# Tarseus/eam-rl4co

Measured on AMD Instinct MI355X. Metric: env-steps/sec (batch x num_loc / s), AttentionModel construction rollout, higher is better.
Workload: dtype f32; 1 GPU; TSP num_loc=100 batch=1024/GPU AM greedy rollout (encoder + cache + decode loop + reward); global_batch=1024, launch=hipGraph replay

## Files before the change

eam_rl4co_amd/csrc/encoder_fused.hip:

```cpp
#include "encoder_fused.hpp"

namespace eamrl {

constexpr int SA = 140;
constexpr int GA = 34;
constexpr int SQ = 66;

struct ALayout {
    float* HB;
    static constexpr int S = SA;
    __device__ float* col(int c) const { return HB + (c & 3) * GA + (c >> 2); }
    __device__ void store4(int row, int q4, float4 v) const
    {
        float* p = HB + row * SA + q4;
        p[0] = v.x; p[GA] = v.y; p[2 * GA] = v.z; p[3 * GA] = v.w;
    }
    __device__ float4 load4(int row, int q4) const
    {
        const float* p = HB + row * SA + q4;
        return make_float4(p[0], p[GA], p[2 * GA], p[3 * GA]);
    }
    __device__ void mirror(int, int, float) const {}
};

#ifdef EAMRL_STAMPS
__device__ unsigned long long g_enc_stamps[24];
#define ESTAMP(i) do { const unsigned long long now_ = __builtin_readcyclecounter(); st_acc[i] += now_ - st_t; st_t = now_; } while (0)
#else
#define ESTAMP(i) do { } while (0)
#endif

__device__ __forceinline__ f32x4 mfma4(float a, float b, f32x4 c) { return __builtin_amdgcn_mfma_f32_16x16x4f32(a, b, c, 0, 0, 0); }

typedef float f32x2v __attribute__((ext_vector_type(2)));
__device__ __forceinline__ float2 lds_read_b64(const float* p)
{
    typedef const volatile __attribute__((address_space(3))) f32x2v* lds_ptr;
    const f32x2v v = *(lds_ptr)(p);
    return make_float2(v.x, v.y);
}

template <int CT>
__device__ __forceinline__ void load_b0(float4 (&b0)[CT], const float* const (&wp)[CT])
{
#pragma unroll
    for (int ct = 0; ct < CT; ++ct) b0[ct] = *reinterpret_cast<const float4*>(wp[ct]);
}

template <int RTW, int CT, int S, bool SWAP, int NRT>
__device__ __forceinline__ void gemm_pass_n(f32x4 (&acc)[RTW][CT], const float* arow, const float* const (&wp)[CT],
                                            int NU, const float4 (&b0)[CT])
{
    constexpr int nrt = NRT;
    float4 bn[CT];
    float2 an0[RTW], an1[RTW];
#pragma unroll
    for (int ct = 0; ct < CT; ++ct) bn[ct] = b0[ct];
#pragma unroll
    for (int rt = 0; rt < RTW; ++rt)
        if (rt < nrt) {
            an0[rt] = lds_read_b64(arow + rt * 16 * S);
            an1[rt] = lds_read_b64(arow + rt * 16 * S + 2);
        }
    for (int u = 0; u < NU; ++u) {
        float4 b[CT];
        float2 a0[RTW], a1[RTW];
#pragma unroll
        for (int ct = 0; ct < CT; ++ct) b[ct] = bn[ct];
#pragma unroll
        for (int rt = 0; rt < RTW; ++rt) { a0[rt] = an0[rt]; a1[rt] = an1[rt]; }
        if (u + 1 < NU) {
#pragma unroll
            for (int ct = 0; ct < CT; ++ct) bn[ct] = *reinterpret_cast<const float4*>(wp[ct] + (u + 1) * 256);
#pragma unroll
            for (int rt = 0; rt < RTW; ++rt)
                if (rt < nrt) {
                    an0[rt] = lds_read_b64(arow + rt * 16 * S + 4 * (u + 1));
                    an1[rt] = lds_read_b64(arow + rt * 16 * S + 4 * (u + 1) + 2);
                }
        }
#pragma unroll
        for (int rt = 0; rt < RTW; ++rt)
            if (rt < nrt) {
#pragma unroll
                for (int ct = 0; ct < CT; ++ct)
                    acc[rt][ct] = SWAP ? mfma4(b[ct].x, a0[rt].x, acc[rt][ct]) : mfma4(a0[rt].x, b[ct].x, acc[rt][ct]);
#pragma unroll
                for (int ct = 0; ct < CT; ++ct)
                    acc[rt][ct] = SWAP ? mfma4(b[ct].y, a0[rt].y, acc[rt][ct]) : mfma4(a0[rt].y, b[ct].y, acc[rt][ct]);
#pragma unroll
                for (int ct = 0; ct < CT; ++ct)
                    acc[rt][ct] = SWAP ? mfma4(b[ct].z, a1[rt].x, acc[rt][ct]) : mfma4(a1[rt].x, b[ct].z, acc[rt][ct]);
#pragma unroll
                for (int ct = 0; ct < CT; ++ct)
                    acc[rt][ct] = SWAP ? mfma4(b[ct].w, a1[rt].y, acc[rt][ct]) : mfma4(a1[rt].y, b[ct].w, acc[rt][ct]);
            }
    }
}

template <int RTW, int CT, int S, bool SWAP = false, int NLOW = RTW>
__device__ __forceinline__ void gemm_pass(f32x4 (&acc)[RTW][CT], const float* arow, int nrt, const float* const (&wp)[CT],
                                          int NU, const float4 (&b0)[CT])
{
    if (NLOW == RTW || nrt == RTW) gemm_pass_n<RTW, CT, S, SWAP, RTW>(acc, arow, wp, NU, b0);
    else gemm_pass_n<RTW, CT, S, SWAP, NLOW>(acc, arow, wp, NU, b0);
}

template <int RTW>
__device__ __forceinline__ void residual_norm_store(const f32x4 (&acc)[RTW][2], float* HB, int row0, int nrt, int cw, int j, int G,
                                                    int norm, const float* cst )
{
#pragma unroll
    for (int ct = 0; ct < 2; ++ct) {
        const int c = 32 * cw + 16 * ct + j;
        const float sc = cst[c], sh = cst[FE + c];
        float* col = HB + (c & 3) * GA + (c >> 2);
#pragma unroll
        for (int rt = 0; rt < RTW; ++rt)
            if (rt < nrt) {
#pragma unroll
                for (int r = 0; r < 4; ++r) {
                    float* p = col + (row0 + 16 * rt + 4 * G + r) * SA;
                    float v = *p + acc[rt][ct][r];
                    if (norm == EAMRL_NORM_BATCH_EVAL) v = fma_(v, sc, sh);
                    *p = v;
                }
            }
    }
}

template <int RTT>
__global__ __launch_bounds__(512, 2) void k_encoder_fused(FusedArgs a)
{
    constexpr int RTA = (RTT + 1) / 2;
    constexpr int RTW = RTA;
    constexpr int ROWS = 16 * RTT;
    constexpr int SV = ROWS + 4;
    extern __shared__ __attribute__((aligned(16))) float lds[];
    float* HB = lds;
    float* QA = HB + ROWS * SA;
    float* KB = QA + ROWS * SQ;
    float* VT = KB + ROWS * SQ;
    float* HID = QA;
    float* CST = VT + 64 * SV;
    static_assert(ROWS * SA <= 2 * ROWS * SQ + 64 * SV, "HID must fit QA | KB | VT");
    const ALayout L{HB};

    const int tid = threadIdx.x, lane = tid & 63;
    const int wv = __builtin_amdgcn_readfirstlane(tid >> 6);
    const int cw = wv & 3, rw = wv >> 2;
    const int j = lane & 15, G = lane >> 4;
    const int M = a.M;
    const int row0 = rw ? 16 * RTA : 0;
    const int nrt = rw ? RTT - RTA : RTA;
    const int64_t inst = blockIdx.x;
#ifdef EAMRL_STAMPS
    unsigned long long st_acc[20] = {0, 0, 0, 0, 0, 0, 0, 0, 0, 0, 0, 0, 0, 0, 0, 0, 0, 0, 0, 0}, st_t = __builtin_readcyclecounter();
#endif

    if (a.h_in) load_h<ROWS>(a.h_in, M, L);
    else init_embedding<ROWS>(a.init, M, L);
    __syncthreads();
    ESTAMP(0);

    for (int layer = 0; layer < a.nlayers; ++layer) {
        const eamrl_encoder_layer& Ly = a.L[layer];
        for (int i = tid; i < NCST; i += blockDim.x) {
            float v;
            if (i < C_BO) v = Ly.bqkv[i];
            else if (i < C_B1) v = Ly.bo[i - C_BO];
            else if (i < C_B2) v = Ly.b1[i - C_B1];
            else if (i < C_N1) v = Ly.b2[i - C_B2];
            else {
                const bool second = i >= C_N2;
                const int k = (i - (second ? C_N2 : C_N1));
                const int c = k & (FE - 1);
                const float* gam = second ? Ly.n2_gamma : Ly.n1_gamma;
                const float* bet = second ? Ly.n2_beta : Ly.n1_beta;
                if (a.norm == EAMRL_NORM_BATCH_EVAL) {
                    const float* mean = second ? Ly.n2_mean : Ly.n1_mean;
                    const float* var = second ? Ly.n2_var : Ly.n1_var;
                    const float sc = gam[c] / __builtin_sqrtf(var[c] + a.eps);
                    const float ms = mean[c] * sc;
                    v = k < FE ? sc : bet[c] - ms;
                } else {
                    v = k < FE ? gam[c] : bet[c];
                }
            }
            CST[i] = v;
        }
        __syncthreads();
        f32x4 acc_o[RTW][2];
#pragma unroll
        for (int ct = 0; ct < 2; ++ct) {
            const float b = CST[C_BO + 32 * cw + 16 * ct + j];
#pragma unroll
            for (int rt = 0; rt < RTW; ++rt) acc_o[rt][ct] = splat4(b);
        }
        for (int hg = 0; hg < 2; ++hg) {
            const float* wp3[2];
            float4 b3[2];
#pragma unroll
            for (int ct = 0; ct < 2; ++ct)
                wp3[ct] = Ly.Wo + ((int64_t)(2 * cw + ct) * (FE / 16) + 4 * hg) * 256 + lane * 4;
            {
                f32x4 acc[RTW][3];
                const int ctq = 4 * hg + cw;
                const float* wp[3];
                float4 b0[3];
#pragma unroll
                for (int x = 0; x < 3; ++x) wp[x] = Ly.Wqkv + ((int64_t)(8 * x + ctq) * (FE / 16)) * 256 + lane * 4;
                load_b0<3>(b0, wp);
#pragma unroll
                for (int x = 0; x < 3; ++x) {
                    const float b = CST[C_BQKV + 16 * (8 * x + ctq) + j];
#pragma unroll
                    for (int rt = 0; rt < RTW; ++rt) acc[rt][x] = splat4(b);
                }
                ESTAMP(16);
                gemm_pass<RTW, 3, SA, false, RTT - RTA>(acc, HB + (row0 + j) * SA + G * GA, nrt, wp, FE / 16, b0);
                ESTAMP(17);
                load_b0<2>(b3, wp3);
                float* qcol = QA + (j & 3) * 16 + 4 * cw + (j >> 2);
                float* kcol = KB + (j & 3) * 16 + 4 * cw + (j >> 2);
                float* vrow = VT + (16 * cw + j) * SV;
#pragma unroll
                for (int rt = 0; rt < RTW; ++rt)
                    if (rt < nrt) {
                        const int rbase = row0 + 16 * rt + 4 * G;
#pragma unroll
                        for (int r = 0; r < 4; ++r) {
                            qcol[(rbase + r) * SQ] = acc[rt][0][r] * 0.25f;
                            kcol[(rbase + r) * SQ] = acc[rt][1][r];
                        }
                        *reinterpret_cast<float4*>(vrow + rbase) =
                            make_float4(acc[rt][2][0], acc[rt][2][1], acc[rt][2][2], acc[rt][2][3]);
                    }
            }
            ESTAMP(1);
            __syncthreads();
            ESTAMP(2);
            {
                const int pi = 4 * (j & 3) + (j >> 2);
                float kf[RTT][4];
#pragma unroll
                for (int kt = 0; kt < RTT; ++kt) {
                    const float* p = KB + (16 * kt + pi) * SQ + G * 16 + 4 * cw;
                    const float2 lo = *reinterpret_cast<const float2*>(p), hi = *reinterpret_cast<const float2*>(p + 2);
                    kf[kt][0] = lo.x; kf[kt][1] = lo.y; kf[kt][2] = hi.x; kf[kt][3] = hi.y;
                }
                float vf[4 * RTT];
                const int NT = (M + 3) >> 2;
                constexpr int FULLT = RTT == 7 ? 4 : RTT == 4 ? 2 : 0;
#pragma unroll
                for (int t = 0; t < 4 * RTT; ++t) vf[t] = (t < NT) ? VT[(16 * cw + j) * SV + 4 * t + G] : 0.0f;
                for (int q = 0; q < nrt; ++q) {
                    const int qrow = row0 + 16 * q + j;
                    const float* qp = QA + qrow * SQ + G * 16 + 4 * cw;
                    const float2 qlo = *reinterpret_cast<const float2*>(qp), qhi = *reinterpret_cast<const float2*>(qp + 2);
                    f32x4 s[RTT];
                    float m = -INFINITY;
#pragma unroll
                    for (int kt = 0; kt < RTT; ++kt) s[kt] = mfma4(kf[kt][0], qlo.x, splat4(0.0f));
#pragma unroll
                    for (int kt = 0; kt < RTT; ++kt) s[kt] = mfma4(kf[kt][1], qlo.y, s[kt]);
#pragma unroll
                    for (int kt = 0; kt < RTT; ++kt) s[kt] = mfma4(kf[kt][2], qhi.x, s[kt]);
#pragma unroll
                    for (int kt = 0; kt < RTT; ++kt) s[kt] = mfma4(kf[kt][3], qhi.y, s[kt]);
#pragma unroll
                    for (int kt = 0; kt < RTT; ++kt) {
                        if (kt >= FULLT && 16 * kt + 16 > M) {
#pragma unroll
                            for (int r = 0; r < 4; ++r)
                                if (16 * kt + 4 * r + G >= M) s[kt][r] = -INFINITY;
                        }
                        m = vmax5_raw(m, s[kt][0], s[kt][1], s[kt][2], s[kt][3]);
                    }
                    {
                        auto r16 = __builtin_amdgcn_permlane16_swap(__float_as_uint(m), __float_as_uint(m), false, false);
                        m = vmax_raw(__uint_as_float(r16[0]), __uint_as_float(r16[1]));
                        auto r32 = __builtin_amdgcn_permlane32_swap(__float_as_uint(m), __float_as_uint(m), false, false);
                        m = vmax_raw(__uint_as_float(r32[0]), __uint_as_float(r32[1]));
                    }
#pragma unroll
                    for (int kt = 0; kt < RTT; ++kt) {
                        f32x2 e01 = (f32x2){s[kt][0], s[kt][1]} - splat2(m), e23 = (f32x2){s[kt][2], s[kt][3]} - splat2(m);
                        d_expf2_nonpos_x2(e01, e23);
                        s[kt] = (f32x4){e01.x, e01.y, e23.x, e23.y};
                    }
                    float zp = s[0][0];
#pragma unroll
                    for (int t = 1; t < 4 * RTT; ++t) zp = zp + s[t >> 2][t & 3];
                    {
                        auto r16 = __builtin_amdgcn_permlane16_swap(__float_as_uint(zp), __float_as_uint(zp), false, false);
                        zp = __uint_as_float(r16[0]) + __uint_as_float(r16[1]);
                        auto r32 = __builtin_amdgcn_permlane32_swap(__float_as_uint(zp), __float_as_uint(zp), false, false);
                        zp = __uint_as_float(r32[0]) + __uint_as_float(r32[1]);
                    }
                    f32x4 o = splat4(0.0f);
#pragma unroll
                    for (int kt = 0; kt < RTT; ++kt)
                        if (kt < FULLT || 16 * kt < M) {
#pragma unroll
                            for (int r = 0; r < 4; ++r) o = mfma4(vf[4 * kt + r], s[kt][r], o);
                        }
                    float* op = QA + qrow * SQ + 4 * cw + G;
#pragma unroll
                    for (int r = 0; r < 4; ++r) op[r * 16] = o[r] / zp;
                }
            }
            ESTAMP(3);
            __syncthreads();
            ESTAMP(4);
            gemm_pass<RTW, 2, SQ, false, RTT - RTA>(acc_o, QA + (row0 + j) * SQ + G * 16, nrt, wp3, 4, b3);
            ESTAMP(5);
            __syncthreads();
            ESTAMP(6);
        }
        residual_norm_store<RTW>(acc_o, HB, row0, nrt, cw, j, G, a.norm, CST + C_N1);
        __syncthreads();
        if (a.norm == EAMRL_NORM_INSTANCE) {
            instance_norm(L, M, a.eps, CST + C_N1);
            __syncthreads();
        }
        ESTAMP(7);
        f32x4 acc_f[RTW][2];
#pragma unroll
        for (int ct = 0; ct < 2; ++ct) {
            const float b = CST[C_B2 + 32 * cw + 16 * ct + j];
#pragma unroll
            for (int rt = 0; rt < RTW; ++rt) acc_f[rt][ct] = splat4(b);
        }
        for (int ch = 0; ch < FF / 128; ++ch) {
            const float* wp5[2];
            float4 b5[2];
#pragma unroll
            for (int ct = 0; ct < 2; ++ct)
                wp5[ct] = Ly.W2 + ((int64_t)(2 * cw + ct) * (FF / 16) + 8 * ch) * 256 + lane * 4;
            {
                f32x4 acc[RTW][2];
                const float* wp[2];
                float4 b0[2];
#pragma unroll
                for (int ct = 0; ct < 2; ++ct) wp[ct] = Ly.W1 + ((int64_t)(8 * ch + 2 * cw + ct) * (FE / 16)) * 256 + lane * 4;
                load_b0<2>(b0, wp);
#pragma unroll
                for (int ct = 0; ct < 2; ++ct) {
                    const float b = CST[C_B1 + 16 * (8 * ch + 2 * cw + ct) + j];
#pragma unroll
                    for (int rt = 0; rt < RTW; ++rt) acc[rt][ct] = splat4(b);
                }
                ESTAMP(14);
                gemm_pass<RTW, 2, SA, false, RTT - RTA>(acc, HB + (row0 + j) * SA + G * GA, nrt, wp, FE / 16, b0);
                ESTAMP(15);
                load_b0<2>(b5, wp5);
#pragma unroll
                for (int ct = 0; ct < 2; ++ct) {
                    const int c = 32 * cw + 16 * ct + j;
                    float* col = HID + (c & 3) * GA + (c >> 2);
#pragma unroll
                    for (int rt = 0; rt < RTW; ++rt)
                        if (rt < nrt) {
#pragma unroll
                            for (int r = 0; r < 4; ++r) {
                                const float v = acc[rt][ct][r];
                                col[(row0 + 16 * rt + 4 * G + r) * SA] = !(v > 0.0f) ? 0.0f : v;
                            }
                        }
                }
            }
            ESTAMP(8);
            __syncthreads();
            ESTAMP(9);
            gemm_pass<RTW, 2, SA, false, RTT - RTA>(acc_f, HID + (row0 + j) * SA + G * GA, nrt, wp5, 8, b5);
            ESTAMP(10);
            __syncthreads();
            ESTAMP(11);
        }
        residual_norm_store<RTW>(acc_f, HB, row0, nrt, cw, j, G, a.norm, CST + C_N2);
        __syncthreads();
        if (a.norm == EAMRL_NORM_INSTANCE) {
            instance_norm(L, M, a.eps, CST + C_N2);
            __syncthreads();
        }
        ESTAMP(12);
    }
    if (a.h_out) store_h(a.h_out, M, L);
    ESTAMP(13);
    if (a.cache.gctx) graph_context(a.cache.Wg, a.cache.gctx, M, L, CST);
    if (a.cache.out) {
        float* STG = QA;
        float* crow = a.cache.out + (inst * (int64_t)M) * a.cache.ld;
        for (int sl = 0; sl <= a.cache.nproj; ++sl) {
            const bool lp = sl == a.cache.nproj;
            f32x4 acc[RTW][2];
            const float* wp[2];
            float4 b0[2];
#pragma unroll
            for (int ct = 0; ct < 2; ++ct)
                wp[ct] = (lp ? a.cache.WoutT : a.cache.Wc + (int64_t)sl * FE * FE) + ((int64_t)(2 * cw + ct) * (FE / 16)) * 256 + lane * 4;
            load_b0<2>(b0, wp);
#pragma unroll
            for (int ct = 0; ct < 2; ++ct)
#pragma unroll
                for (int rt = 0; rt < RTW; ++rt) acc[rt][ct] = splat4(0.0f);
            if (lp) __syncthreads();
            gemm_pass<RTW, 2, SA, true, RTT - RTA>(acc, (lp ? STG : HB) + (row0 + j) * SA + G * GA, nrt, wp, FE / 16, b0);
#pragma unroll
            for (int rt = 0; rt < RTW; ++rt)
                if (rt < nrt) {
                    const int node = row0 + 16 * rt + j;
#pragma unroll
                    for (int ct = 0; ct < 2; ++ct) {
                        const int c = 32 * cw + 16 * ct + 4 * G;
                        const f32x4 v = acc[rt][ct];
                        if (node < M)
                            *reinterpret_cast<float4*>(crow + (int64_t)node * a.cache.ld + sl * FE + c) = make_float4(v[0], v[1], v[2], v[3]);
                        if (sl == 2) {
                            float* p = STG + node * SA + (c >> 2);
                            p[0] = v[0]; p[GA] = v[1]; p[2 * GA] = v[2]; p[3 * GA] = v[3];
                        }
                    }
                }
        }
    }
#ifdef EAMRL_STAMPS
    if (lane == 0) {
        for (int i = 0; i < 20; ++i) atomicAdd(&g_enc_stamps[i], st_acc[i]);
        atomicAdd(&g_enc_stamps[20], 1ull);
    }
#endif
}

__global__ void k_pack_mfma_b(const float* __restrict__ W, float* __restrict__ Wp, int N, int K)
{
    const int64_t idx = (int64_t)blockIdx.x * blockDim.x + threadIdx.x;
    if (idx >= (int64_t)N * K) return;
    const int q = (int)(idx & 3), l = (int)((idx >> 2) & 63);
    const int64_t blk = idx >> 8;
    const int u = (int)(blk % (K / 16)), ct = (int)(blk / (K / 16));
    const int j = l & 15, g = l >> 4;
    Wp[idx] = W[(int64_t)(16 * ct + j) * K + 16 * u + 4 * q + g];
}

int launch_pack_mfma_b(const float* W, float* Wp, int N, int K, hipStream_t st)
{
    const int64_t n = (int64_t)N * K;
    hipLaunchKernelGGL(k_pack_mfma_b, dim3((unsigned)((n + 255) / 256)), dim3(256), 0, st, W, Wp, N, K);
    return hipGetLastError() == hipSuccess ? 0 : EAMRL_E_LAUNCH;
}

#ifdef EAMRL_STAMPS
extern "C" __attribute__((visibility("default"))) int eamrl_debug_read_enc_stamps(unsigned long long* out, int reset)
{
    if (hipMemcpyFromSymbol(out, HIP_SYMBOL(g_enc_stamps), sizeof(g_enc_stamps)) != hipSuccess) return -1;
    if (reset) {
        unsigned long long z[24] = {0};
        if (hipMemcpyToSymbol(HIP_SYMBOL(g_enc_stamps), z, sizeof(z)) != hipSuccess) return -1;
    }
    return 0;
}
#endif

bool encoder_fused_supports(int M, int E, int H, int FFdim, int nlayers)
{
    return M >= 1 && M <= 112 && E == FE && H == FH && FFdim == FF && nlayers >= 1 && nlayers <= MAX_FUSED_LAYERS;
}

int launch_encoder_fused(const float* h_in, float* h_out, int64_t B, int M, int nlayers, int norm, float eps,
                         const eamrl_encoder_layer* layers, const eamrl_encoder_cache* cache, const eamrl_encoder_init* init,
                         int dtype, hipStream_t st)
{
    if (B <= 0) return 0;
    FusedArgs a = {};
    a.h_in = init ? nullptr : h_in; a.h_out = h_out; a.M = M; a.nlayers = nlayers; a.norm = norm; a.eps = eps;
    if (cache) {
        a.cache = *cache;
        if (!cache->Wg || !cache->gctx) a.cache.Wg = a.cache.gctx = nullptr;
    }
    if (init) a.init = *init;
    for (int l = 0; l < nlayers; ++l) a.L[l] = layers[l];
    if (dtype != DTYPE_F32) return launch_encoder_fused16(a, B, dtype, st);
    return launch_fused(a, B, st, [](auto rtt) {
        constexpr int RTT = decltype(rtt)::value, ROWS = 16 * RTT;
        return FusedVariant{k_encoder_fused<RTT>, ((size_t)ROWS * SA + 2 * (size_t)ROWS * SQ + 64 * (size_t)(ROWS + 4) + NCST) * sizeof(float)};
    });
}

}
```

Baseline: 49.11 million env-steps/s.

## Handle ragged encoder row tail with 4x4 MFMA tiles interleaved into main GEMMs

When the node count leaves a small remainder in the last 16-row tile, the fused encoder kernel now computes the full tiles over one fewer row tile. The leftover rows go through 4x4x1 MFMA accumulations that are interleaved into the main GEMM loops, assigned to otherwise lighter waves. This avoids wasted 16x16 MFMA work on padding rows in the QKV, output projection, FFN and cache projection GEMMs. In exchange it adds extra LDS reads, register pressure, template variants and a zero-init pass over the attention buffers.

```diff
diff --git a/eam_rl4co_amd/csrc/encoder_fused.hip b/eam_rl4co_amd/csrc/encoder_fused.hip
--- a/eam_rl4co_amd/csrc/encoder_fused.hip
+++ b/eam_rl4co_amd/csrc/encoder_fused.hip
@@ -47,12 +47,18 @@
     for (int ct = 0; ct < CT; ++ct) b0[ct] = *reinterpret_cast<const float4*>(wp[ct]);
 }
 
-template <int RTW, int CT, int S, bool SWAP, int NRT>
+__device__ __forceinline__ f32x4 mfma1(float a, float b, f32x4 c) { return __builtin_amdgcn_mfma_f32_4x4x1f32(a, b, c, 0, 0, 0); }
+
+__device__ __forceinline__ float comp4(const float4 v, int q) { return q == 0 ? v.x : q == 1 ? v.y : q == 2 ? v.z : v.w; }
+
+template <int RTW, int CT, int S, bool SWAP, int NRT, int NQ, int TG>
 __device__ __forceinline__ void gemm_pass_n(f32x4 (&acc)[RTW][CT], const float* arow, const float* const (&wp)[CT],
-                                            int NU, const float4 (&b0)[CT])
+                                            int NU, const float4 (&b0)[CT], f32x4 (&tacc)[NQ ? NQ : 1], const float* tarow,
+                                            const float* twp)
 {
     constexpr int nrt = NRT;
-    float4 bn[CT];
+    constexpr int NQA = NQ ? NQ : 1, NT = 16 * NQ, NG = NRT ? 4 * NRT : 1;
+    float4 bn[CT], tbn[4];
     float2 an0[RTW], an1[RTW];
 #pragma unroll
     for (int ct = 0; ct < CT; ++ct) bn[ct] = b0[ct];
@@ -62,13 +68,21 @@
             an0[rt] = lds_read_b64(arow + rt * 16 * S);
             an1[rt] = lds_read_b64(arow + rt * 16 * S + 2);
         }
+    if (NQ) {
+#pragma unroll
+        for (int g = 0; g < 4; ++g) tbn[g] = *reinterpret_cast<const float4*>(twp + 64 * g);
+    }
     for (int u = 0; u < NU; ++u) {
-        float4 b[CT];
-        float2 a0[RTW], a1[RTW];
+        float4 b[CT], tb[4];
+        float2 a0[RTW], a1[RTW], ta[NQA][4][2];
 #pragma unroll
         for (int ct = 0; ct < CT; ++ct) b[ct] = bn[ct];
 #pragma unroll
         for (int rt = 0; rt < RTW; ++rt) { a0[rt] = an0[rt]; a1[rt] = an1[rt]; }
+        if (NQ) {
+#pragma unroll
+            for (int g = 0; g < 4; ++g) tb[g] = tbn[g];
+        }
         if (u + 1 < NU) {
 #pragma unroll
             for (int ct = 0; ct < CT; ++ct) bn[ct] = *reinterpret_cast<const float4*>(wp[ct] + (u + 1) * 256);
@@ -78,38 +92,74 @@
                     an0[rt] = lds_read_b64(arow + rt * 16 * S + 4 * (u + 1));
                     an1[rt] = lds_read_b64(arow + rt * 16 * S + 4 * (u + 1) + 2);
                 }
-        }
+            if (NQ) {
+#pragma unroll
+                for (int g = 0; g < 4; ++g) tbn[g] = *reinterpret_cast<const float4*>(twp + (u + 1) * 256 + 64 * g);
+            }
+        }
+        if (NQ) {
+#pragma unroll
+            for (int qd = 0; qd < NQA; ++qd)
+#pragma unroll
+                for (int g = 0; g < 4; ++g) {
+                    ta[qd][g][0] = lds_read_b64(tarow + qd * 4 * S + g * TG + 4 * u);
+                    ta[qd][g][1] = lds_read_b64(tarow + qd * 4 * S + g * TG + 4 * u + 2);
+                }
+        }
+#define EAMRL_TAIL_STEPS(lo, hi)                                                                                          \
+        _Pragma("unroll") for (int i = 0; i < NT; ++i)                                                                    \
+            if (i >= (lo) && i < (hi)) {                                                                                  \
+                const int kk = i / NQA, qd = i % NQA, q = kk >> 2, g = kk & 3;                                            \
+                const float2 av = ta[qd][g][q >> 1];                                                                      \
+                tacc[qd] = mfma1((q & 1) ? av.y : av.x, comp4(tb[g], q), tacc[qd]);                                       \
+            }
 #pragma unroll
         for (int rt = 0; rt < RTW; ++rt)
             if (rt < nrt) {
 #pragma unroll
-                for (int ct = 0; ct < CT; ++ct)
-                    acc[rt][ct] = SWAP ? mfma4(b[ct].x, a0[rt].x, acc[rt][ct]) : mfma4(a0[rt].x, b[ct].x, acc[rt][ct]);
-#pragma unroll
-                for (int ct = 0; ct < CT; ++ct)
-                    acc[rt][ct] = SWAP ? mfma4(b[ct].y, a0[rt].y, acc[rt][ct]) : mfma4(a0[rt].y, b[ct].y, acc[rt][ct]);
-#pragma unroll
-                for (int ct = 0; ct < CT; ++ct)
-                    acc[rt][ct] = SWAP ? mfma4(b[ct].z, a1[rt].x, acc[rt][ct]) : mfma4(a1[rt].x, b[ct].z, acc[rt][ct]);
-#pragma unroll
-                for (int ct = 0; ct < CT; ++ct)
-                    acc[rt][ct] = SWAP ? mfma4(b[ct].w, a1[rt].y, acc[rt][ct]) : mfma4(a1[rt].y, b[ct].w, acc[rt][ct]);
-            }
-    }
-}
-
-template <int RTW, int CT, int S, bool SWAP = false, int NLOW = RTW>
+                for (int q = 0; q < 4; ++q) {
+                    const float av = q == 0 ? a0[rt].x : q == 1 ? a0[rt].y : q == 2 ? a1[rt].x : a1[rt].y;
+#pragma unroll
+                    for (int ct = 0; ct < CT; ++ct)
+                        acc[rt][ct] = SWAP ? mfma4(comp4(b[ct], q), av, acc[rt][ct]) : mfma4(av, comp4(b[ct], q), acc[rt][ct]);
+                    if (NQ) { EAMRL_TAIL_STEPS(((4 * rt + q) * NT) / NG, ((4 * rt + q + 1) * NT) / NG) }
+                }
+            }
+        if (NQ && NRT == 0) { EAMRL_TAIL_STEPS(0, NT) }
+#undef EAMRL_TAIL_STEPS
+    }
+}
+
+template <int RTW, int CT, int S, bool SWAP = false, int NLOW = RTW, int NQ = 0, int TG = 0>
 __device__ __forceinline__ void gemm_pass(f32x4 (&acc)[RTW][CT], const float* arow, int nrt, const float* const (&wp)[CT],
-                                          int NU, const float4 (&b0)[CT])
-{
-    if (NLOW == RTW || nrt == RTW) gemm_pass_n<RTW, CT, S, SWAP, RTW>(acc, arow, wp, NU, b0);
-    else gemm_pass_n<RTW, CT, S, SWAP, NLOW>(acc, arow, wp, NU, b0);
-}
-
-template <int RTW>
+                                          int NU, const float4 (&b0)[CT], bool tail, f32x4 (&tacc)[NQ ? NQ : 1],
+                                          const float* tarow, const float* twp)
+{
+    f32x4 none[1];
+    if (NQ > 0 && tail) gemm_pass_n<RTW, CT, S, SWAP, NLOW, NQ, TG>(acc, arow, wp, NU, b0, tacc, tarow, twp);
+    else if (NLOW == RTW || nrt == RTW) gemm_pass_n<RTW, CT, S, SWAP, RTW, 0, 0>(acc, arow, wp, NU, b0, none, nullptr, nullptr);
+    else gemm_pass_n<RTW, CT, S, SWAP, NLOW, 0, 0>(acc, arow, wp, NU, b0, none, nullptr, nullptr);
+}
+
+template <int RTW, int NQ>
 __device__ __forceinline__ void residual_norm_store(const f32x4 (&acc)[RTW][2], float* HB, int row0, int nrt, int cw, int j, int G,
-                                                    int norm, const float* cst )
-{
+                                                    int norm, const float* cst ,
+                                                    bool tail, const f32x4 (&tacc)[NQ ? NQ : 1], int trow, int tg, int lane)
+{
+    if (NQ > 0 && tail) {
+        const int c = 64 * tg + lane;
+        const float sc = cst[c], sh = cst[FE + c];
+        float* col = HB + (c & 3) * GA + (c >> 2);
+#pragma unroll
+        for (int qd = 0; qd < NQ; ++qd)
+#pragma unroll
+            for (int r = 0; r < 4; ++r) {
+                float* p = col + (trow + 4 * qd + r) * SA;
+                float v = *p + tacc[qd][r];
+                if (norm == EAMRL_NORM_BATCH_EVAL) v = fma_(v, sc, sh);
+                *p = v;
+            }
+    }
 #pragma unroll
     for (int ct = 0; ct < 2; ++ct) {
         const int c = 32 * cw + 16 * ct + j;
@@ -129,11 +179,15 @@
     }
 }
 
-template <int RTT>
+template <int RTT, int NQ>
 __global__ __launch_bounds__(512, 2) void k_encoder_fused(FusedArgs a)
 {
     constexpr int RTA = (RTT + 1) / 2;
-    constexpr int RTW = RTA;
+    constexpr int RTF = NQ ? RTT - 1 : RTT;
+    constexpr int RTG = (RTF + 1) / 2;
+    constexpr int RTW = RTG;
+    constexpr int NQA = NQ ? NQ : 1;
+    constexpr int TROW = 16 * RTF;
     constexpr int ROWS = 16 * RTT;
     constexpr int SV = ROWS + 4;
     extern __shared__ __attribute__((aligned(16))) float lds[];
@@ -153,6 +207,14 @@
     const int M = a.M;
     const int row0 = rw ? 16 * RTA : 0;
     const int nrt = rw ? RTT - RTA : RTA;
+    const int grow0 = rw ? 16 * RTG : 0;
+    const int gnrt = rw ? RTF - RTG : RTG;
+    const bool tail1 = NQ > 0 && rw == 1 && cw < 3;
+    const bool tail4 = NQ > 0 && rw == 1 && cw < 2;
+    const bool tail2 = NQ > 0 && rw == 1 && cw >= 2;
+    const int tg2 = 3 - cw;
+    const int tw4 = (lane & 15) * 4;
+    const int tct = lane >> 4;
     const int64_t inst = blockIdx.x;
 #ifdef EAMRL_STAMPS
     unsigned long long st_acc[20] = {0, 0, 0, 0, 0, 0, 0, 0, 0, 0, 0, 0, 0, 0, 0, 0, 0, 0, 0, 0}, st_t = __builtin_readcyclecounter();
@@ -160,6 +222,9 @@
 
     if (a.h_in) load_h<ROWS>(a.h_in, M, L);
     else init_embedding<ROWS>(a.init, M, L);
+    if (NQ) {
+        for (int i = tid; i < 2 * ROWS * SQ + 64 * SV; i += 512) QA[i] = 0.0f;
+    }
     __syncthreads();
     ESTAMP(0);
 
@@ -197,6 +262,12 @@
 #pragma unroll
             for (int rt = 0; rt < RTW; ++rt) acc_o[rt][ct] = splat4(b);
         }
+        f32x4 tacc_o[NQA];
+        if (tail2) {
+            const float b = CST[C_BO + 64 * tg2 + lane];
+#pragma unroll
+            for (int qd = 0; qd < NQA; ++qd) tacc_o[qd] = splat4(b);
+        }
         for (int hg = 0; hg < 2; ++hg) {
             const float* wp3[2];
             float4 b3[2];
@@ -217,8 +288,17 @@
 #pragma unroll
                     for (int rt = 0; rt < RTW; ++rt) acc[rt][x] = splat4(b);
                 }
+                f32x4 tacc[NQA];
+                const float* twp = Ly.Wqkv;
+                if (tail1) {
+                    twp = Ly.Wqkv + ((int64_t)(8 * cw + 4 * hg + tct) * (FE / 16)) * 256 + tw4;
+                    const float b = CST[C_BQKV + 128 * cw + 64 * hg + lane];
+#pragma unroll
+                    for (int qd = 0; qd < NQA; ++qd) tacc[qd] = splat4(b);
+                }
                 ESTAMP(16);
-                gemm_pass<RTW, 3, SA, false, RTT - RTA>(acc, HB + (row0 + j) * SA + G * GA, nrt, wp, FE / 16, b0);
+                gemm_pass<RTW, 3, SA, false, RTF - RTG, NQ, GA>(acc, HB + (grow0 + j) * SA + G * GA, gnrt, wp, FE / 16, b0,
+                                                                tail1, tacc, HB + (TROW + (lane & 3)) * SA, twp);
                 ESTAMP(17);
                 load_b0<2>(b3, wp3);
                 float* qcol = QA + (j & 3) * 16 + 4 * cw + (j >> 2);
@@ -226,8 +306,8 @@
                 float* vrow = VT + (16 * cw + j) * SV;
 #pragma unroll
                 for (int rt = 0; rt < RTW; ++rt)
-                    if (rt < nrt) {
-                        const int rbase = row0 + 16 * rt + 4 * G;
+                    if (rt < gnrt) {
+                        const int rbase = grow0 + 16 * rt + 4 * G;
 #pragma unroll
                         for (int r = 0; r < 4; ++r) {
                             qcol[(rbase + r) * SQ] = acc[rt][0][r] * 0.25f;
@@ -236,6 +316,19 @@
                         *reinterpret_cast<float4*>(vrow + rbase) =
                             make_float4(acc[rt][2][0], acc[rt][2][1], acc[rt][2][2], acc[rt][2][3]);
                     }
+                if (tail1) {
+                    float* tcol = (cw == 0 ? QA : KB) + (lane & 3) * 16 + (lane >> 2);
+#pragma unroll
+                    for (int qd = 0; qd < NQA; ++qd) {
+                        const f32x4 v = tacc[qd];
+                        if (cw == 2) {
+                            *reinterpret_cast<float4*>(VT + lane * SV + TROW + 4 * qd) = make_float4(v[0], v[1], v[2], v[3]);
+                        } else {
+#pragma unroll
+                            for (int r = 0; r < 4; ++r) tcol[(TROW + 4 * qd + r) * SQ] = cw == 0 ? v[r] * 0.25f : v[r];
+                        }
+                    }
+                }
             }
             ESTAMP(1);
             __syncthreads();
@@ -313,12 +406,14 @@
             ESTAMP(3);
             __syncthreads();
             ESTAMP(4);
-            gemm_pass<RTW, 2, SQ, false, RTT - RTA>(acc_o, QA + (row0 + j) * SQ + G * 16, nrt, wp3, 4, b3);
+            gemm_pass<RTW, 2, SQ, false, RTF - RTG, NQ, 16>(acc_o, QA + (grow0 + j) * SQ + G * 16, gnrt, wp3, 4, b3, tail2, tacc_o,
+                                                            QA + (TROW + (lane & 3)) * SQ,
+                                                            Ly.Wo + ((int64_t)(4 * tg2 + tct) * (FE / 16) + 4 * hg) * 256 + tw4);
             ESTAMP(5);
             __syncthreads();
             ESTAMP(6);
         }
-        residual_norm_store<RTW>(acc_o, HB, row0, nrt, cw, j, G, a.norm, CST + C_N1);
+        residual_norm_store<RTW, NQ>(acc_o, HB, grow0, gnrt, cw, j, G, a.norm, CST + C_N1, tail2, tacc_o, TROW, tg2, lane);
         __syncthreads();
         if (a.norm == EAMRL_NORM_INSTANCE) {
             instance_norm(L, M, a.eps, CST + C_N1);
@@ -331,6 +426,12 @@
             const float b = CST[C_B2 + 32 * cw + 16 * ct + j];
 #pragma unroll
             for (int rt = 0; rt < RTW; ++rt) acc_f[rt][ct] = splat4(b);
+        }
+        f32x4 tacc_f[NQA];
+        if (tail2) {
+            const float b = CST[C_B2 + 64 * tg2 + lane];
+#pragma unroll
+            for (int qd = 0; qd < NQA; ++qd) tacc_f[qd] = splat4(b);
         }
         for (int ch = 0; ch < FF / 128; ++ch) {
             const float* wp5[2];
@@ -351,8 +452,16 @@
 #pragma unroll
                     for (int rt = 0; rt < RTW; ++rt) acc[rt][ct] = splat4(b);
                 }
+                f32x4 tacc[NQA];
+                if (tail4) {
+                    const float b = CST[C_B1 + 128 * ch + 64 * cw + lane];
+#pragma unroll
+                    for (int qd = 0; qd < NQA; ++qd) tacc[qd] = splat4(b);
+                }
                 ESTAMP(14);
-                gemm_pass<RTW, 2, SA, false, RTT - RTA>(acc, HB + (row0 + j) * SA + G * GA, nrt, wp, FE / 16, b0);
+                gemm_pass<RTW, 2, SA, false, RTF - RTG, NQ, GA>(acc, HB + (grow0 + j) * SA + G * GA, gnrt, wp, FE / 16, b0, tail4, tacc,
+                                                                HB + (TROW + (lane & 3)) * SA,
+                                                                Ly.W1 + ((int64_t)(8 * ch + 4 * cw + tct) * (FE / 16)) * 256 + tw4);
                 ESTAMP(15);
                 load_b0<2>(b5, wp5);
 #pragma unroll
@@ -361,24 +470,37 @@
                     float* col = HID + (c & 3) * GA + (c >> 2);
 #pragma unroll
                     for (int rt = 0; rt < RTW; ++rt)
-                        if (rt < nrt) {
+                        if (rt < gnrt) {
 #pragma unroll
                             for (int r = 0; r < 4; ++r) {
                                 const float v = acc[rt][ct][r];
-                                col[(row0 + 16 * rt + 4 * G + r) * SA] = !(v > 0.0f) ? 0.0f : v;
+                                col[(grow0 + 16 * rt + 4 * G + r) * SA] = !(v > 0.0f) ? 0.0f : v;
                             }
+                        }
+                }
+                if (tail4) {
+                    const int c = 64 * cw + lane;
+                    float* col = HID + (c & 3) * GA + (c >> 2);
+#pragma unroll
+                    for (int qd = 0; qd < NQA; ++qd)
+#pragma unroll
+                        for (int r = 0; r < 4; ++r) {
+                            const float v = tacc[qd][r];
+                            col[(TROW + 4 * qd + r) * SA] = !(v > 0.0f) ? 0.0f : v;
                         }
                 }
             }
             ESTAMP(8);
             __syncthreads();
             ESTAMP(9);
-            gemm_pass<RTW, 2, SA, false, RTT - RTA>(acc_f, HID + (row0 + j) * SA + G * GA, nrt, wp5, 8, b5);
+            gemm_pass<RTW, 2, SA, false, RTF - RTG, NQ, GA>(acc_f, HID + (grow0 + j) * SA + G * GA, gnrt, wp5, 8, b5, tail2, tacc_f,
+                                                            HID + (TROW + (lane & 3)) * SA,
+                                                            Ly.W2 + ((int64_t)(4 * tg2 + tct) * (FF / 16) + 8 * ch) * 256 + tw4);
             ESTAMP(10);
             __syncthreads();
             ESTAMP(11);
         }
-        residual_norm_store<RTW>(acc_f, HB, row0, nrt, cw, j, G, a.norm, CST + C_N2);
+        residual_norm_store<RTW, NQ>(acc_f, HB, grow0, gnrt, cw, j, G, a.norm, CST + C_N2, tail2, tacc_f, TROW, tg2, lane);
         __syncthreads();
         if (a.norm == EAMRL_NORM_INSTANCE) {
             instance_norm(L, M, a.eps, CST + C_N2);
@@ -405,12 +527,18 @@
             for (int ct = 0; ct < 2; ++ct)
 #pragma unroll
                 for (int rt = 0; rt < RTW; ++rt) acc[rt][ct] = splat4(0.0f);
+            f32x4 tacc[NQA];
+#pragma unroll
+            for (int qd = 0; qd < NQA; ++qd) tacc[qd] = splat4(0.0f);
             if (lp) __syncthreads();
-            gemm_pass<RTW, 2, SA, true, RTT - RTA>(acc, (lp ? STG : HB) + (row0 + j) * SA + G * GA, nrt, wp, FE / 16, b0);
+            gemm_pass<RTW, 2, SA, true, RTF - RTG, NQ, GA>(acc, (lp ? STG : HB) + (grow0 + j) * SA + G * GA, gnrt, wp, FE / 16, b0, tail2,
+                                                           tacc, (lp ? STG : HB) + (TROW + (lane & 3)) * SA,
+                                                           (lp ? a.cache.WoutT : a.cache.Wc + (int64_t)sl * FE * FE) +
+                                                               ((int64_t)(4 * tg2 + tct) * (FE / 16)) * 256 + tw4);
 #pragma unroll
             for (int rt = 0; rt < RTW; ++rt)
-                if (rt < nrt) {
-                    const int node = row0 + 16 * rt + j;
+                if (rt < gnrt) {
+                    const int node = grow0 + 16 * rt + j;
 #pragma unroll
                     for (int ct = 0; ct < 2; ++ct) {
                         const int c = 32 * cw + 16 * ct + 4 * G;
@@ -423,6 +551,18 @@
                         }
                     }
                 }
+            if (tail2) {
+                const int c = 64 * tg2 + lane;
+#pragma unroll
+                for (int qd = 0; qd < NQA; ++qd)
+#pragma unroll
+                    for (int r = 0; r < 4; ++r) {
+                        const int node = TROW + 4 * qd + r;
+                        const float v = tacc[qd][r];
+                        if (node < M) crow[(int64_t)node * a.cache.ld + sl * FE + c] = v;
+                        if (sl == 2) STG[node * SA + (c & 3) * GA + (c >> 2)] = v;
+                    }
+            }
         }
     }
 #ifdef EAMRL_STAMPS
@@ -482,9 +622,15 @@
     if (init) a.init = *init;
     for (int l = 0; l < nlayers; ++l) a.L[l] = layers[l];
     if (dtype != DTYPE_F32) return launch_encoder_fused16(a, B, dtype, st);
-    return launch_fused(a, B, st, [](auto rtt) {
+    return launch_fused(a, B, st, [M](auto rtt) {
         constexpr int RTT = decltype(rtt)::value, ROWS = 16 * RTT;
-        return FusedVariant{k_encoder_fused<RTT>, ((size_t)ROWS * SA + 2 * (size_t)ROWS * SQ + 64 * (size_t)(ROWS + 4) + NCST) * sizeof(float)};
+        const int t = M - 16 * (RTT - 1);
+        constexpr int FITS = RTT == 7 ? 1 : RTT == 4 ? 2 : 3;
+        const int nq = t >= 1 && t <= 4 * FITS ? (t + 3) / 4 : 0;
+        void (*kernel)(FusedArgs) = nq == 1 ? k_encoder_fused<RTT, 1> : k_encoder_fused<RTT, 0>;
+        if constexpr (FITS >= 2) if (nq == 2) kernel = k_encoder_fused<RTT, 2>;
+        if constexpr (FITS >= 3) if (nq == 3) kernel = k_encoder_fused<RTT, 3>;
+        return FusedVariant{kernel, ((size_t)ROWS * SA + 2 * (size_t)ROWS * SQ + 64 * (size_t)(ROWS + 4) + NCST) * sizeof(float)};
     });
 }
 
```

After: 49.95 million env-steps/s, median of 6. +1.7%, better.
